# castacks/UniCeption

Hardware: AMD Instinct MI355X
Metric: image-pairs/sec fwd, ViT-L/16 two-view 512x512 (encoder + CroCo decoder + dpt heads + adaptor) (higher is better)
Workload: dtype bf16; 1 GPU; BASELINE configs[1]: ViT-L/16 CroCo encoder + 12-block CroCo decoder + dpt head, 512x512 pairs, forward, random-init weights; pairs_per_gpu=128, img=512, head=dpt, encoder=croco, attention=bf16, hipgraph=False, parallelism=dp1 (independent pairs per rank, no data-path collective)

## Files before the change

### uniception_amd/csrc/elementwise.hip

```cpp
#include "vec_access.h"
#include <type_traits>
#include "knobs.h"

template <typename TO>
__global__ void patch_gather_kernel(const float* __restrict__ img, typename TO::storage* __restrict__ cols, int B,
                                    int Cin, int H, int W, int P, int64_t items) {
    const int h = H / P, w = W / P;
    const int P4 = P / 4;
    for (int64_t it = (int64_t)blockIdx.x * blockDim.x + threadIdx.x; it < items; it += (int64_t)gridDim.x * blockDim.x) {
        int64_t r = it;
        const int v4 = (int)(r % P4); r /= P4;
        const int u = (int)(r % P); r /= P;
        const int c = (int)(r % Cin); r /= Cin;
        const int j = (int)(r % w); r /= w;
        const int i = (int)(r % h);
        const int b = (int)(r / h);
        const float4_t px = *reinterpret_cast<const float4_t*>(
            img + (((int64_t)b * Cin + c) * H + (int64_t)i * P + u) * W + (int64_t)j * P + v4 * 4);
        typename TO::storage* o = cols + it * 4;
        TO::store(o + 0, px.x); TO::store(o + 1, px.y); TO::store(o + 2, px.z); TO::store(o + 3, px.w);
    }
}

template <typename TO>
__global__ void patch_gather_scalar_kernel(const float* __restrict__ img, typename TO::storage* __restrict__ cols, int B,
                                           int Cin, int H, int W, int P, int64_t n) {
    const int h = H / P, w = W / P;
    for (int64_t it = (int64_t)blockIdx.x * blockDim.x + threadIdx.x; it < n; it += (int64_t)gridDim.x * blockDim.x) {
        int64_t r = it;
        const int v = (int)(r % P); r /= P;
        const int u = (int)(r % P); r /= P;
        const int c = (int)(r % Cin); r /= Cin;
        const int j = (int)(r % w); r /= w;
        const int i = (int)(r % h);
        const int b = (int)(r / h);
        TO::store(cols + it, img[(((int64_t)b * Cin + c) * H + (int64_t)i * P + u) * W + (int64_t)j * P + v]);
    }
}

extern "C" int uc_patch_gather(const float* img, void* cols, int out_dtype, int B, int Cin, int H, int W, int P,
                               uc_stream_t stream) {
    UC_REQUIRE(img && cols, "uc_patch_gather: null pointer");
    UC_REQUIRE(B > 0 && Cin > 0 && P > 0 && H % P == 0 && W % P == 0, "uc_patch_gather: H,W must be multiples of the patch size");
    hipStream_t st = (hipStream_t)stream;
    const bool quad = (P % 4 == 0) && (W % 4 == 0) && ((uintptr_t)img % 16 == 0);
    if (!quad) {
        const int64_t n = (int64_t)B * Cin * H * W;
        UC_DISPATCH("uc_patch_gather", out_dtype,
                    hipLaunchKernelGGL((patch_gather_scalar_kernel<Tag>), dim3(EW_GRID(n)), dim3(256), 0, st, img, (Tag::storage*)cols, B, Cin, H, W, P, n));
        UC_CHECK_LAUNCH("uc_patch_gather");
        return UC_OK;
    }
    const int64_t items = (int64_t)B * Cin * H * W / 4;
    UC_DISPATCH("uc_patch_gather", out_dtype,
                hipLaunchKernelGGL((patch_gather_kernel<Tag>), dim3(EW_GRID(items)), dim3(256), 0, st, img, (Tag::storage*)cols, B, Cin, H, W, P, items));
    UC_CHECK_LAUNCH("uc_patch_gather");
    return UC_OK;
}

template <typename TI, typename TO>
__global__ __launch_bounds__(256) void transpose2d_kernel(const typename TI::storage* __restrict__ src,
                                                          typename TO::storage* __restrict__ dst, int R, int S) {
    __shared__ float tile[32][33];
    const int64_t boff = (int64_t)blockIdx.z * R * S;
    const int s0 = blockIdx.x * 32, r0 = blockIdx.y * 32;
    const int tx = threadIdx.x & 31, ty = threadIdx.x >> 5;
#pragma unroll
    for (int k = 0; k < 4; ++k) {
        const int r = r0 + ty + 8 * k, s = s0 + tx;
        if (r < R && s < S) tile[ty + 8 * k][tx] = TI::load(src + boff + (int64_t)r * S + s);
    }
    __syncthreads();
#pragma unroll
    for (int k = 0; k < 4; ++k) {
        const int s = s0 + ty + 8 * k, r = r0 + tx;
        if (r < R && s < S) TO::store(dst + boff + (int64_t)s * R + r, tile[tx][ty + 8 * k]);
    }
}

template <typename TI, typename TO>
static void launch_transpose(const void* src, void* dst, int Bn, int R, int S, hipStream_t st) {
    hipLaunchKernelGGL((transpose2d_kernel<TI, TO>), dim3((S + 31) / 32, (R + 31) / 32, Bn), dim3(256), 0, st,
                       (const typename TI::storage*)src, (typename TO::storage*)dst, R, S);
}

static int dispatch_transpose(const char* name, const void* src, int sd, void* dst, int dd, int Bn, int R, int S,
                              hipStream_t st) {
    UC_REQUIRE(src && dst, "%s: null pointer", name);
    UC_REQUIRE(Bn > 0 && R > 0 && S > 0 && Bn <= 65535 && (R + 31) / 32 <= 65535, "%s: bad shape", name);
    if (sd == UC_F32 && dd == UC_F32) launch_transpose<F32Tag, F32Tag>(src, dst, Bn, R, S, st);
    else if (sd == UC_F32 && dd == UC_BF16) launch_transpose<F32Tag, BF16Tag>(src, dst, Bn, R, S, st);
    else if (sd == UC_BF16 && dd == UC_F32) launch_transpose<BF16Tag, F32Tag>(src, dst, Bn, R, S, st);
    else if (sd == UC_BF16 && dd == UC_BF16) launch_transpose<BF16Tag, BF16Tag>(src, dst, Bn, R, S, st);
    else if (sd == UC_F32 && dd == UC_F16) launch_transpose<F32Tag, F16Tag>(src, dst, Bn, R, S, st);
    else if (sd == UC_F16 && dd == UC_F32) launch_transpose<F16Tag, F32Tag>(src, dst, Bn, R, S, st);
    else if (sd == UC_BF16 && dd == UC_F16) launch_transpose<BF16Tag, F16Tag>(src, dst, Bn, R, S, st);
    else { uc_set_error("%s: unsupported dtypes %d -> %d", name, sd, dd); return UC_ERR_BAD_ARG; }
    UC_CHECK_LAUNCH(name);
    return UC_OK;
}

extern "C" int uc_nchw_to_nhwc(const void* src, int src_dtype, void* dst, int dst_dtype, int B, int C, int H, int W,
                               uc_stream_t stream) {
    return dispatch_transpose("uc_nchw_to_nhwc", src, src_dtype, dst, dst_dtype, B, C, H * W, (hipStream_t)stream);
}
extern "C" int uc_nhwc_to_nchw(const void* src, int src_dtype, void* dst, int dst_dtype, int B, int C, int H, int W,
                               uc_stream_t stream) {
    return dispatch_transpose("uc_nhwc_to_nchw", src, src_dtype, dst, dst_dtype, B, H * W, C, (hipStream_t)stream);
}

template <typename TI, typename TO>
__global__ void convert_kernel(const typename TI::storage* __restrict__ s, typename TO::storage* __restrict__ d, int64_t n, int* __restrict__ sat_flag, int vec) {
    constexpr bool TO_F16 = sizeof(typename TO::storage) == 2 && !std::is_same<TO, BF16Tag>::value;
    const int64_t n8 = vec ? n >> 3 : 0;
    float amax = 0.f;
    for (int64_t i = (int64_t)blockIdx.x * blockDim.x + threadIdx.x; i < n8; i += (int64_t)gridDim.x * blockDim.x) {
        float v[8];
        if constexpr (sizeof(typename TI::storage) == 4) {
            const float4_t a = *reinterpret_cast<const float4_t*>(s + i * 8), b = *reinterpret_cast<const float4_t*>(s + i * 8 + 4);
            v[0] = a.x; v[1] = a.y; v[2] = a.z; v[3] = a.w; v[4] = b.x; v[5] = b.y; v[6] = b.z; v[7] = b.w;
        } else {
            typename TI::storage raw[8];
            *reinterpret_cast<uint4*>(raw) = *reinterpret_cast<const uint4*>(s + i * 8);
#pragma unroll
            for (int k = 0; k < 8; ++k) v[k] = TI::load(raw + k);
        }
        if constexpr (TO_F16) {
#pragma unroll
            for (int k = 0; k < 8; ++k) amax = uc_amax(amax, fabsf(v[k]));
        }
        if constexpr (sizeof(typename TO::storage) == 4) {
            *reinterpret_cast<float4_t*>(d + i * 8) = (float4_t){v[0], v[1], v[2], v[3]};
            *reinterpret_cast<float4_t*>(d + i * 8 + 4) = (float4_t){v[4], v[5], v[6], v[7]};
        } else {
            typename TO::storage raw[8];
#pragma unroll
            for (int k = 0; k < 8; ++k) TO::store(raw + k, v[k]);
            *reinterpret_cast<uint4*>(d + i * 8) = *reinterpret_cast<const uint4*>(raw);
        }
    }
    for (int64_t i = (n8 << 3) + (int64_t)blockIdx.x * blockDim.x + threadIdx.x; i < n; i += (int64_t)gridDim.x * blockDim.x) {
        const float v = TI::load(s + i);
        if constexpr (TO_F16) amax = uc_amax(amax, fabsf(v));
        TO::store(d + i, v);
    }
    if constexpr (TO_F16) {
        if (sat_flag && !(amax <= UC_F16_MAX)) atomicOr(sat_flag, 1);
    }
}

extern "C" int uc_convert(const void* src, int sd, void* dst, int dd, int64_t n, int* sat_flag, uc_stream_t stream) {
    UC_REQUIRE(src && dst && n >= 0, "uc_convert: bad argument");
    if (n == 0) return UC_OK;
    const int vec = ((uintptr_t)src % 16 == 0 && (uintptr_t)dst % 16 == 0) ? 1 : 0;
    hipStream_t st = (hipStream_t)stream;
    const dim3 g(EW_GRID(vec ? (n + 7) / 8 : n)), b(256);
    if (sd == UC_F32 && dd == UC_BF16) hipLaunchKernelGGL((convert_kernel<F32Tag, BF16Tag>), g, b, 0, st, (const float*)src, (bf16_t*)dst, n, sat_flag, vec);
    else if (sd == UC_BF16 && dd == UC_F32) hipLaunchKernelGGL((convert_kernel<BF16Tag, F32Tag>), g, b, 0, st, (const bf16_t*)src, (float*)dst, n, sat_flag, vec);
    else if (sd == UC_F32 && dd == UC_F32) hipLaunchKernelGGL((convert_kernel<F32Tag, F32Tag>), g, b, 0, st, (const float*)src, (float*)dst, n, sat_flag, vec);
    else if (sd == UC_BF16 && dd == UC_BF16) hipLaunchKernelGGL((convert_kernel<BF16Tag, BF16Tag>), g, b, 0, st, (const bf16_t*)src, (bf16_t*)dst, n, sat_flag, vec);
    else if (sd == UC_F32 && dd == UC_F16) hipLaunchKernelGGL((convert_kernel<F32Tag, F16Tag>), g, b, 0, st, (const float*)src, (unsigned short*)dst, n, sat_flag, vec);
    else if (sd == UC_F16 && dd == UC_F32) hipLaunchKernelGGL((convert_kernel<F16Tag, F32Tag>), g, b, 0, st, (const unsigned short*)src, (float*)dst, n, sat_flag, vec);
    else if (sd == UC_BF16 && dd == UC_F16) hipLaunchKernelGGL((convert_kernel<BF16Tag, F16Tag>), g, b, 0, st, (const bf16_t*)src, (unsigned short*)dst, n, sat_flag, vec);
    else { uc_set_error("uc_convert: unsupported dtypes %d -> %d", sd, dd); return UC_ERR_BAD_ARG; }
    UC_CHECK_LAUNCH("uc_convert");
    return UC_OK;
}

__global__ void add_view_pe_kernel(float* __restrict__ x, const float* __restrict__ pe, int64_t B, int L, int T, int V, int C4) {
    const int64_t n = B * (int64_t)V * T * C4;
    for (int64_t i = (int64_t)blockIdx.x * blockDim.x + threadIdx.x; i < n; i += (int64_t)gridDim.x * blockDim.x) {
        const int c = (int)(i % C4);
        const int64_t r = i / C4;
        const int64_t bv = r / T;
        const int v = (int)(bv % V);
        const int64_t b = bv / V;
        float4_t* px = reinterpret_cast<float4_t*>(x + ((b * L + (int64_t)v * T + (r - bv * T)) * C4 + c) * 4);
        *px = *px + *reinterpret_cast<const float4_t*>(pe + ((int64_t)v * C4 + c) * 4);
    }
}

extern "C" int uc_add_view_pe(float* x, const float* pe, int64_t B, int L, int T, int V, int C, uc_stream_t stream) {
    UC_REQUIRE(x && pe && B >= 0 && L > 0 && T > 0 && V > 0 && (int64_t)V * T <= L && C > 0 && C % 4 == 0, "uc_add_view_pe: bad argument");
    UC_REQUIRE((uintptr_t)x % 16 == 0 && (uintptr_t)pe % 16 == 0, "uc_add_view_pe: 16-byte alignment");
    const int64_t n = B * (int64_t)V * T * (C / 4);
    if (n == 0) return UC_OK;
    hipLaunchKernelGGL(add_view_pe_kernel, dim3(EW_GRID(n)), dim3(256), 0, (hipStream_t)stream, x, pe, B, L, T, V, C / 4);
    UC_CHECK_LAUNCH("uc_add_view_pe");
    return UC_OK;
}

__global__ void split_bf16x3_kernel(const float* __restrict__ x, bf16_t* __restrict__ out, int64_t rows, int C8, int relu) {
    const int64_t n = rows * C8;
    for (int64_t i = (int64_t)blockIdx.x * blockDim.x + threadIdx.x; i < n; i += (int64_t)gridDim.x * blockDim.x) {
        const int64_t r = i / C8;
        const int c = (int)(i - r * C8);
        const float4_t* src = reinterpret_cast<const float4_t*>(x + (r * C8 + c) * 8);
        float v[8];
        const float4_t a = src[0], b = src[1];
        v[0] = a.x; v[1] = a.y; v[2] = a.z; v[3] = a.w; v[4] = b.x; v[5] = b.y; v[6] = b.z; v[7] = b.w;
        unsigned hi[4], lo[4];
#pragma unroll
        for (int k = 0; k < 4; ++k) {
            float p = v[2 * k], q = v[2 * k + 1];
            if (relu) { p = fmaxf(p, 0.f); q = fmaxf(q, 0.f); }
            const unsigned h = pack_bf16x2(p, q);
            hi[k] = h;
            lo[k] = pack_bf16x2(p - __uint_as_float(h << 16), q - __uint_as_float(h & 0xffff0000u));
        }
        bf16_t* dst = out + r * (int64_t)C8 * 24 + c * 8;
        const uint4 H = (uint4){hi[0], hi[1], hi[2], hi[3]};
        *reinterpret_cast<uint4*>(dst) = H;
        *reinterpret_cast<uint4*>(dst + (int64_t)C8 * 8) = H;
        *reinterpret_cast<uint4*>(dst + (int64_t)C8 * 16) = (uint4){lo[0], lo[1], lo[2], lo[3]};
    }
}

extern "C" int uc_split_bf16x3(const float* x, void* out, int64_t rows, int C, int relu, uc_stream_t stream) {
    UC_REQUIRE(x && out && rows >= 0 && C > 0 && C % 8 == 0, "uc_split_bf16x3: C must be a positive multiple of 8");
    UC_REQUIRE((uintptr_t)x % 16 == 0 && (uintptr_t)out % 16 == 0, "uc_split_bf16x3: 16-byte alignment");
    if (rows == 0) return UC_OK;
    const int64_t n = rows * (C / 8);
    hipLaunchKernelGGL(split_bf16x3_kernel, dim3(EW_GRID(n)), dim3(256), 0, (hipStream_t)stream, x, (bf16_t*)out, rows, C / 8, relu);
    UC_CHECK_LAUNCH("uc_split_bf16x3");
    return UC_OK;
}

template <typename Tag>
__global__ void bilinear_kernel(const typename Tag::storage* __restrict__ src, typename Tag::storage* __restrict__ dst,
                                int B, int Hi, int Wi, int C, int Ho, int Wo, int ch, int cw, float sy, float sx) {
    const unsigned C8 = (unsigned)C / 8u;
    const unsigned t = blockIdx.x * blockDim.x + threadIdx.x;
    if (t >= (unsigned)cw * C8) return;
    const unsigned ox = t / C8, c8 = t - ox * C8;
    const int oy = blockIdx.y, b = blockIdx.z;
    const float fy = sy * (float)oy, fx = sx * (float)ox;
    const int y0 = (int)fy, x0 = (int)fx;
    const int y1 = min(y0 + 1, Hi - 1), x1 = min(x0 + 1, Wi - 1);
    const float ly = fy - (float)y0, lx = fx - (float)x0;
    const float hy = 1.f - ly, hx = 1.f - lx;
    const typename Tag::storage* base = src + (int64_t)b * Hi * Wi * C + c8 * 8;
    const Vec8 p00 = vec_load8<Tag>(base + ((int64_t)y0 * Wi + x0) * C);
    const Vec8 p01 = vec_load8<Tag>(base + ((int64_t)y0 * Wi + x1) * C);
    const Vec8 p10 = vec_load8<Tag>(base + ((int64_t)y1 * Wi + x0) * C);
    const Vec8 p11 = vec_load8<Tag>(base + ((int64_t)y1 * Wi + x1) * C);
    Vec8 o;
#pragma unroll
    for (int e = 0; e < 8; ++e)
        o.v[e] = hy * (hx * p00.v[e] + lx * p01.v[e]) + ly * (hx * p10.v[e] + lx * p11.v[e]);
    vec_store8<Tag>(dst + (((int64_t)b * ch + oy) * cw) * C + (int64_t)t * 8, o);
}

template <typename Tag, int R>
__global__ void bilinear_rows_kernel(const typename Tag::storage* __restrict__ src, typename Tag::storage* __restrict__ dst,
                                     int B, int Hi, int Wi, int C, int Ho, int Wo, int ch, int cw, float sy, float sx) {
    constexpr int RIN = R / 2 + 2;
    const unsigned C8 = (unsigned)C / 8u;
    const unsigned t = blockIdx.x * blockDim.x + threadIdx.x;
    if (t >= (unsigned)cw * C8) return;
    const unsigned ox = t / C8, c8 = t - ox * C8;
    const int oy = R * blockIdx.y, b = blockIdx.z;
    const float fx = sx * (float)ox;
    const int x0 = (int)fx;
    const int x1 = min(x0 + 1, Wi - 1);
    const float lx = fx - (float)x0, hx = 1.f - lx;
    const int ya = (int)(sy * (float)oy);
    const typename Tag::storage* base = src + (int64_t)b * Hi * Wi * C + c8 * 8;
    float h[RIN][8];
#pragma unroll
    for (int i = 0; i < RIN; ++i) {
        const int64_t y = min(ya + i, Hi - 1);
        const Vec8 p0 = vec_load8<Tag>(base + (y * Wi + x0) * C), p1 = vec_load8<Tag>(base + (y * Wi + x1) * C);
#pragma unroll
        for (int e = 0; e < 8; ++e) h[i][e] = hx * p0.v[e] + lx * p1.v[e];
    }
#pragma unroll
    for (int k = 0; k < R; ++k) {
        if (oy + k >= ch) break;
        const float fy = sy * (float)(oy + k);
        const int y0 = (int)fy;
        const float ly = fy - (float)y0, hy = 1.f - ly;
        const int rel = y0 - ya;
        Vec8 o;
#pragma unroll
        for (int e = 0; e < 8; ++e) {
            float top = h[0][e], bot = h[1][e];
#pragma unroll
            for (int i = 1; i < RIN - 1; ++i) { top = rel == i ? h[i][e] : top; bot = rel == i ? h[i + 1][e] : bot; }
            o.v[e] = hy * top + ly * bot;
        }
        vec_store8<Tag>(dst + (((int64_t)b * ch + oy + k) * cw) * C + (int64_t)t * 8, o);
    }
}

extern "C" int uc_bilinear_nhwc(const void* src, void* dst, int dtype, int B, int Hi, int Wi, int C, int Ho, int Wo,
                                int crop_h, int crop_w, uc_stream_t stream) {
    UC_REQUIRE(src && dst, "uc_bilinear_nhwc: null pointer");
    UC_REQUIRE(B > 0 && Hi > 0 && Wi > 0 && Ho > 0 && Wo > 0 && C > 0 && C % 8 == 0, "uc_bilinear_nhwc: bad shape (C must be a multiple of 8)");
    UC_REQUIRE(crop_h > 0 && crop_h <= Ho && crop_w > 0 && crop_w <= Wo, "uc_bilinear_nhwc: bad crop");
    const float sy = Ho > 1 ? (float)(Hi - 1) / (float)(Ho - 1) : 0.f;
    const float sx = Wo > 1 ? (float)(Wi - 1) / (float)(Wo - 1) : 0.f;
    UC_REQUIRE(crop_h <= 65535 && B <= 65535 && (int64_t)crop_w * (C / 8) < ((int64_t)1 << 31), "uc_bilinear_nhwc: shape exceeds the launch grid");
    const dim3 grid((unsigned)(((int64_t)crop_w * (C / 8) + 255) / 256), (unsigned)crop_h, (unsigned)B);
    hipStream_t st = (hipStream_t)stream;
    const int rows2 = uc_knobs().bilinear_rows2;
    if (rows2 && sy <= 0.5f && (dtype == UC_BF16 || dtype == UC_F16)) {
#define UC_BL_ROWS(TAG, R)                                                                                                           \
    hipLaunchKernelGGL((bilinear_rows_kernel<TAG, R>), dim3(grid.x, (unsigned)((crop_h + R - 1) / R), (unsigned)B), dim3(256), 0, st, \
                       (const TAG::storage*)src, (TAG::storage*)dst, B, Hi, Wi, C, Ho, Wo, crop_h, crop_w, sy, sx)
        if (dtype == UC_F16) UC_BL_ROWS(F16Tag, 4);
        else if (rows2 == 4) UC_BL_ROWS(BF16Tag, 4);
        else UC_BL_ROWS(BF16Tag, 2);
#undef UC_BL_ROWS
        UC_CHECK_LAUNCH("uc_bilinear_nhwc");
        return UC_OK;
    }
    UC_DISPATCH_F16("uc_bilinear_nhwc", dtype,
                    hipLaunchKernelGGL((bilinear_kernel<Tag>), grid, dim3(256), 0, st, (const Tag::storage*)src, (Tag::storage*)dst, B, Hi, Wi, C, Ho, Wo, crop_h, crop_w, sy, sx));
    UC_CHECK_LAUNCH("uc_bilinear_nhwc");
    return UC_OK;
}

template <typename Tag>
__global__ void convt_scatter_kernel(const typename Tag::storage* __restrict__ src, typename Tag::storage* __restrict__ dst,
                                     int B, int h, int w, int k, int Cout, int64_t items) {
    const int C8 = Cout / 8;
    for (int64_t it = (int64_t)blockIdx.x * blockDim.x + threadIdx.x; it < items; it += (int64_t)gridDim.x * blockDim.x) {
        int64_t r = it;
        const int c8 = (int)(r % C8); r /= C8;
        const int X = (int)(r % (k * w)); r /= (k * w);
        const int Y = (int)(r % (k * h));
        const int b = (int)(r / (k * h));
        const int i = Y / k, u = Y % k, j = X / k, v = X % k;
        const int64_t srow = ((int64_t)b * h + i) * w + j;
        const Vec8 x = vec_load8<Tag>(src + srow * ((int64_t)k * k * Cout) + (int64_t)(u * k + v) * Cout + c8 * 8);
        vec_store8<Tag>(dst + it * 8, x);
    }
}

extern "C" int uc_convt_scatter(const void* src, void* dst, int dtype, int B, int h, int w, int k, int Cout,
                                uc_stream_t stream) {
    UC_REQUIRE(src && dst, "uc_convt_scatter: null pointer");
    UC_REQUIRE(B > 0 && h > 0 && w > 0 && k > 0 && Cout > 0 && Cout % 8 == 0, "uc_convt_scatter: bad shape (Cout must be a multiple of 8)");
    const int64_t items = (int64_t)B * h * w * k * k * (Cout / 8);
    hipStream_t st = (hipStream_t)stream;
    UC_DISPATCH_F16("uc_convt_scatter", dtype,
                    hipLaunchKernelGGL((convt_scatter_kernel<Tag>), dim3(EW_GRID(items)), dim3(256), 0, st, (const Tag::storage*)src, (Tag::storage*)dst, B, h, w, k, Cout, items));
    UC_CHECK_LAUNCH("uc_convt_scatter");
    return UC_OK;
}

template <typename Tag>
__global__ void pixel_shuffle_kernel(const typename Tag::storage* __restrict__ src, float* __restrict__ dst, int B, int h,
                                     int w, int P, int Cout, int64_t n) {
    const int Wd = P * w, Hd = P * h;
    for (int64_t it = (int64_t)blockIdx.x * blockDim.x + threadIdx.x; it < n; it += (int64_t)gridDim.x * blockDim.x) {
        int64_t r = it;
        const int X = (int)(r % Wd); r /= Wd;
        const int Y = (int)(r % Hd); r /= Hd;
        const int c = (int)(r % Cout);
        const int b = (int)(r / Cout);
        const int i = Y / P, u = Y % P, j = X / P, v = X % P;
        const int64_t srow = ((int64_t)b * h + i) * w + j;
        dst[it] = Tag::load(src + srow * ((int64_t)Cout * P * P) + (int64_t)c * P * P + u * P + v);
    }
}

extern "C" int uc_pixel_shuffle(const void* src, int src_dtype, float* dst, int B, int h, int w, int P, int Cout,
                                uc_stream_t stream) {
    UC_REQUIRE(src && dst && B > 0 && h > 0 && w > 0 && P > 0 && Cout > 0, "uc_pixel_shuffle: bad argument");
    const int64_t n = (int64_t)B * Cout * P * h * P * w;
    hipStream_t st = (hipStream_t)stream;
    UC_DISPATCH_F16("uc_pixel_shuffle", src_dtype,
                    hipLaunchKernelGGL((pixel_shuffle_kernel<Tag>), dim3(EW_GRID(n)), dim3(256), 0, st, (const Tag::storage*)src, dst, B, h, w, P, Cout, n));
    UC_CHECK_LAUNCH("uc_pixel_shuffle");
    return UC_OK;
}

__global__ void pointmap_adaptor_kernel(const float* __restrict__ x, int64_t sb, int64_t sc, int64_t sp,
                                        float* __restrict__ pts, float* __restrict__ conf, int64_t HW, int64_t n,
                                        float vmin, float vspan) {
    for (int64_t it = (int64_t)blockIdx.x * blockDim.x + threadIdx.x; it < n; it += (int64_t)gridDim.x * blockDim.x) {
        const int64_t b = it / HW, pix = it % HW;
        const float* px = x + b * sb + pix * sp;
        const float X = px[0], Y = px[sc], Z = px[2 * sc], Cf = px[3 * sc];
        const float d = sqrtf(X * X + Y * Y + Z * Z);
        const float s = expm1f(d) / fmaxf(d, 1e-8f);
        pts[it * 3 + 0] = X * s;
        pts[it * 3 + 1] = Y * s;
        pts[it * 3 + 2] = Z * s;
        conf[it] = vmin + fminf(expf(Cf), vspan);
    }
}

extern "C" int uc_pointmap_adaptor(const float* x, int64_t x_sb, int64_t x_sc, int64_t x_sp, float* pts, float* conf,
                                   int B, int H, int W, float conf_vmin, float conf_vmax, uc_stream_t stream) {
    UC_REQUIRE(x && pts && conf && B > 0 && H > 0 && W > 0, "uc_pointmap_adaptor: bad argument");
    const int64_t n = (int64_t)B * H * W;
    hipLaunchKernelGGL(pointmap_adaptor_kernel, dim3(EW_GRID(n)), dim3(256), 0, (hipStream_t)stream, x, x_sb, x_sc, x_sp,
                       pts, conf, (int64_t)H * W, n, conf_vmin, conf_vmax - conf_vmin);
    UC_CHECK_LAUNCH("uc_pointmap_adaptor");
    return UC_OK;
}

template <typename Tag>
__global__ __launch_bounds__(256) void conv1x1_to4_kernel(const typename Tag::storage* __restrict__ feat,
                                                          const float* __restrict__ w, const float* __restrict__ bias,
                                                          float* __restrict__ out, int64_t npix, int Cin) {
    __shared__ float ws[4][256];
    for (int i = threadIdx.x; i < 4 * Cin; i += blockDim.x) ws[i / Cin][i % Cin] = w[i];
    __syncthreads();
    for (int64_t pix = (int64_t)blockIdx.x * blockDim.x + threadIdx.x; pix < npix; pix += (int64_t)gridDim.x * blockDim.x) {
        float a0 = bias[0], a1 = bias[1], a2 = bias[2], a3 = bias[3];
        const typename Tag::storage* f = feat + pix * Cin;
        for (int c = 0; c < Cin; c += 8) {
            const Vec8 x = vec_load8<Tag>(f + c);
#pragma unroll
            for (int e = 0; e < 8; ++e) {
                a0 = fmaf(x.v[e], ws[0][c + e], a0);
                a1 = fmaf(x.v[e], ws[1][c + e], a1);
                a2 = fmaf(x.v[e], ws[2][c + e], a2);
                a3 = fmaf(x.v[e], ws[3][c + e], a3);
            }
        }
        *reinterpret_cast<float4_t*>(out + pix * 4) = (float4_t){a0, a1, a2, a3};
    }
}

template <typename Tag, int C8>
__global__ __launch_bounds__(256) void conv1x1_to4_coop_kernel(const typename Tag::storage* __restrict__ feat,
                                                               const float* __restrict__ w, const float* __restrict__ bias,
                                                               float* __restrict__ out, int64_t npix) {
    constexpr int Cin = C8 * 8;
    constexpr int PPB = 256 / C8;
    const int chunk = threadIdx.x % C8, pl = threadIdx.x / C8;
    float wr[4][8];
#pragma unroll
    for (int o = 0; o < 4; ++o)
#pragma unroll
        for (int e = 0; e < 8; ++e) wr[o][e] = w[o * Cin + chunk * 8 + e];
    const float4_t b4 = *reinterpret_cast<const float4_t*>(bias);
    for (int64_t pix = (int64_t)blockIdx.x * PPB + pl; pix < npix; pix += (int64_t)gridDim.x * PPB) {
        const Vec8 x = vec_load8<Tag>(feat + pix * Cin + chunk * 8);
        float a[4] = {0.f, 0.f, 0.f, 0.f};
#pragma unroll
        for (int e = 0; e < 8; ++e) {
            a[0] = fmaf(x.v[e], wr[0][e], a[0]);
            a[1] = fmaf(x.v[e], wr[1][e], a[1]);
            a[2] = fmaf(x.v[e], wr[2][e], a[2]);
            a[3] = fmaf(x.v[e], wr[3][e], a[3]);
        }
#pragma unroll
        for (int off = C8 / 2; off > 0; off >>= 1) {
#pragma unroll
            for (int o = 0; o < 4; ++o) a[o] += __shfl_xor(a[o], off, 64);
        }
        if (chunk == 0)
            *reinterpret_cast<float4_t*>(out + pix * 4) = (float4_t){a[0] + b4.x, a[1] + b4.y, a[2] + b4.z, a[3] + b4.w};
    }
}

template <typename Tag>
static bool launch_conv1x1_to4_coop(const void* feat, const float* w, const float* b, float* out, int64_t npix, int Cin, hipStream_t st) {
    const int C8 = Cin / 8;
// ... 366 lines not shown
```

### uniception_amd/csrc/error.hip

```cpp
#include "common.h"
#include "knobs.h"

#include <mutex>
#include <stdlib.h>
#include <string.h>

static thread_local char g_uc_err[512] = {0};

void uc_set_error(const char* fmt, ...) {
    va_list ap;
    va_start(ap, fmt);
    vsnprintf(g_uc_err, sizeof(g_uc_err), fmt, ap);
    va_end(ap);
}

extern "C" const char* uc_last_error(void) { return g_uc_err; }
extern "C" int uc_abi_version(void) { return UC_ABI_VERSION; }

#ifdef UC_DIAG
extern "C" const char* uc_build_flavor(void) { return "diag"; }
#else
extern "C" const char* uc_build_flavor(void) { return "release"; }
#endif

#define UC_ATTN_RS_DEFAULT 0
static UcKnobs g_knobs;
static std::once_flag g_knobs_once;
std::atomic<int> g_uc_gemm_variant{-3};
std::atomic<int> g_uc_gemm_stagger{-1};
std::atomic<int> g_uc_attn_rs{UC_ATTN_RS_DEFAULT};
std::atomic<int> g_uc_attn_p64{1};
std::atomic<int> g_uc_attn_bwd64{1};
std::atomic<int> g_uc_conv_rows{1};
std::atomic<int> g_uc_conv_rows_flat{1};
std::atomic<int> g_uc_small_m_split{2048};

static int env_int(const char* name, int dflt) {
    const char* e = getenv(name);
    return e ? atoi(e) : dflt;
}

const UcKnobs& uc_knobs() {
    std::call_once(g_knobs_once, [] {
        g_knobs.gemm_group_m = env_int("UC_GEMM_GROUP_M", 4);
        if (g_knobs.gemm_group_m < 1) g_knobs.gemm_group_m = 1;
        g_knobs.gemm_4wave = env_int("UC_GEMM_4WAVE", 3);
        g_knobs.attn_prio = env_int("UC_ATTN_PRIO", 0);
        g_knobs.bilinear_rows2 = env_int("UC_BILINEAR_ROWS2", 4);
        g_knobs.ln_nt = env_int("UC_LN_NT", -1);
#ifdef UC_DIAG
        g_knobs.gemm_dbg = env_int("UC_GEMM_DBG", 0);
        g_knobs.attn_dbg = env_int("UC_ATTN_DBG", 0);
        g_knobs.gemm_trace = env_int("UC_GEMM_TRACE", 0);
#endif
        g_uc_gemm_variant.store(env_int("UC_GEMM_VARIANT", -3));
        g_uc_gemm_stagger.store(env_int("UC_GEMM_STAGGER", -1));
        g_uc_attn_rs.store(env_int("UC_ATTN_RS", UC_ATTN_RS_DEFAULT));
        g_uc_attn_p64.store(env_int("UC_ATTN_P64", 1));
        g_uc_attn_bwd64.store(env_int("UC_ATTN_BWD64", 1));
        g_uc_conv_rows.store(env_int("UC_CONV_ROWS", 1));
        g_uc_conv_rows_flat.store(env_int("UC_CONV_ROWS_FLAT", 1));
        g_uc_small_m_split.store(env_int("UC_GEMM_SMALLM", 2048));
    });
    return g_knobs;
}

extern "C" int uc_tuning_set(const char* name, int value) {
    UC_REQUIRE(name, "uc_tuning_set: null name");
    (void)uc_knobs();
    if (!strcmp(name, "gemm_variant")) {
        UC_REQUIRE(value == -3 || value == -1 || (value >= 0 && value <= 4) || value == 6 || value == 7, "uc_tuning_set: gemm_variant must be -3 (automatic), -1, 0..4, 6 or 7 (got %d)", value);
        g_uc_gemm_variant.store(value);
    } else if (!strcmp(name, "gemm_stagger")) {
        UC_REQUIRE(value >= -1 && value <= 100000, "uc_tuning_set: gemm_stagger out of range (%d)", value);
        g_uc_gemm_stagger.store(value);
    } else if (!strcmp(name, "attn_role_split")) {
        UC_REQUIRE(value == 0 || value == 1, "uc_tuning_set: attn_role_split must be 0 or 1 (got %d)", value);
        g_uc_attn_rs.store(value);
    } else if (!strcmp(name, "attn_p64")) {
        UC_REQUIRE(value >= 0 && value <= 2, "uc_tuning_set: attn_p64 must be 0 (never), 1 (policy) or 2 (wherever the shape allows) (got %d)", value);
        g_uc_attn_p64.store(value);
    } else if (!strcmp(name, "attn_bwd64")) {
        UC_REQUIRE(value >= 0 && value <= 2, "uc_tuning_set: attn_bwd64 must be 0 (never), 1 (policy) or 2 (always) (got %d)", value);
        g_uc_attn_bwd64.store(value);
    } else if (!strcmp(name, "small_m_split")) {
        UC_REQUIRE(value >= 0, "uc_tuning_set: small_m_split is the smallest K a small-M launch splits in two for (0: never) (got %d)", value);
        g_uc_small_m_split.store(value);
    } else if (!strcmp(name, "conv_rows")) {
        UC_REQUIRE(value >= 0 && value <= 3, "uc_tuning_set: conv_rows must be 0 (implicit GEMM everywhere), 1 (row-walking kernels where they win), 2 (the 256-pixel row-walking kernel wherever the shape allows) or 3 (the eight-wave 512-pixel one wherever the shape allows) (got %d)", value);
        g_uc_conv_rows.store(value);
    } else if (!strcmp(name, "conv_rows_flat")) {
        UC_REQUIRE(value == 0 || value == 1, "uc_tuning_set: conv_rows_flat must be 0 (the eight-wave row kernel only on maps whose rows tile 512 pixels) or 1 (its flat form on every other map too) (got %d)", value);
        g_uc_conv_rows_flat.store(value);
    } else {
        uc_set_error("uc_tuning_set: unknown knob '%s' (run-time switchable: gemm_variant, gemm_stagger, attn_role_split, attn_p64, attn_bwd64, conv_rows, conv_rows_flat, small_m_split; everything else is read from the environment once, see csrc/knobs.h)", name);
        return UC_ERR_BAD_ARG;
    }
    return UC_OK;
}

extern "C" int uc_tuning_get(const char* name, int* value) {
    UC_REQUIRE(name && value, "uc_tuning_get: null argument");
    (void)uc_knobs();
    if (!strcmp(name, "gemm_variant")) *value = g_uc_gemm_variant.load();
    else if (!strcmp(name, "gemm_stagger")) *value = g_uc_gemm_stagger.load();
    else if (!strcmp(name, "attn_role_split")) *value = g_uc_attn_rs.load();
    else if (!strcmp(name, "attn_p64")) *value = g_uc_attn_p64.load();
    else if (!strcmp(name, "attn_bwd64")) *value = g_uc_attn_bwd64.load();
    else if (!strcmp(name, "conv_rows")) *value = g_uc_conv_rows.load();
    else if (!strcmp(name, "conv_rows_flat")) *value = g_uc_conv_rows_flat.load();
    else if (!strcmp(name, "small_m_split")) *value = g_uc_small_m_split.load();
    else { uc_set_error("uc_tuning_get: unknown knob '%s'", name); return UC_ERR_BAD_ARG; }
    return UC_OK;
}
```

### uniception_amd/csrc/knobs.h

```cpp
#pragma once
#include <atomic>

struct UcKnobs {
    int gemm_group_m;
    int gemm_4wave;
    int attn_prio;
    int bilinear_rows2;
    int ln_nt;
#ifdef UC_DIAG
    int gemm_dbg;
    int attn_dbg;
    int gemm_trace;
#endif
};
const UcKnobs& uc_knobs();

extern std::atomic<int> g_uc_gemm_variant;
extern std::atomic<int> g_uc_gemm_stagger;
extern std::atomic<int> g_uc_small_m_split;
extern std::atomic<int> g_uc_conv_rows;
extern std::atomic<int> g_uc_conv_rows_flat;
extern std::atomic<int> g_uc_attn_p64;
extern std::atomic<int> g_uc_attn_bwd64;
extern std::atomic<int> g_uc_attn_rs;

#ifdef UC_DIAG
#define UC_DBG(p, bits) ((p).dbg & (bits))
#define UC_TRACE(p) ((p).trace)
#else
#define UC_DBG(p, bits) (0)
#define UC_TRACE(p) ((unsigned long long*)nullptr)
#endif
```

### uniception_amd/csrc/vec_access.h

```cpp
#pragma once
#include "common.h"

struct Vec8 { float v[8]; };

__device__ __forceinline__ unsigned pack_f16x2(float lo, float hi) {
    const float2v_t v = {uc_sat_f16(lo), uc_sat_f16(hi)};
    return __builtin_bit_cast(unsigned, __builtin_convertvector(v, half2v_t));
}
__device__ __forceinline__ void unpack_f16x2(unsigned u, float& lo, float& hi) {
    const float2v_t v = __builtin_convertvector(__builtin_bit_cast(half2v_t, u), float2v_t);
    lo = v.x; hi = v.y;
}
__device__ __forceinline__ float4_t unpack_bf16x4(uint2 r) {
    return (float4_t){__uint_as_float(r.x << 16), __uint_as_float(r.x & 0xffff0000u), __uint_as_float(r.y << 16), __uint_as_float(r.y & 0xffff0000u)};
}

template <typename Tag> __device__ __forceinline__ Vec8 vec_load8(const typename Tag::storage* p);
template <> __device__ __forceinline__ Vec8 vec_load8<F32Tag>(const float* p) {
    Vec8 r;
    const float4_t a = *reinterpret_cast<const float4_t*>(p);
    const float4_t b = *reinterpret_cast<const float4_t*>(p + 4);
    r.v[0] = a.x; r.v[1] = a.y; r.v[2] = a.z; r.v[3] = a.w; r.v[4] = b.x; r.v[5] = b.y; r.v[6] = b.z; r.v[7] = b.w;
    return r;
}
template <> __device__ __forceinline__ Vec8 vec_load8<BF16Tag>(const bf16_t* p) {
    Vec8 r;
    const uint4 u = *reinterpret_cast<const uint4*>(p);
    r.v[0] = __uint_as_float(u.x << 16); r.v[1] = __uint_as_float(u.x & 0xffff0000u);
    r.v[2] = __uint_as_float(u.y << 16); r.v[3] = __uint_as_float(u.y & 0xffff0000u);
    r.v[4] = __uint_as_float(u.z << 16); r.v[5] = __uint_as_float(u.z & 0xffff0000u);
    r.v[6] = __uint_as_float(u.w << 16); r.v[7] = __uint_as_float(u.w & 0xffff0000u);
    return r;
}
template <> __device__ __forceinline__ Vec8 vec_load8<F16Tag>(const unsigned short* p) {
    Vec8 r;
    const uint4 u = *reinterpret_cast<const uint4*>(p);
    unpack_f16x2(u.x, r.v[0], r.v[1]); unpack_f16x2(u.y, r.v[2], r.v[3]);
    unpack_f16x2(u.z, r.v[4], r.v[5]); unpack_f16x2(u.w, r.v[6], r.v[7]);
    return r;
}

template <typename Tag> __device__ __forceinline__ void vec_store8(typename Tag::storage* p, const Vec8& r);
template <> __device__ __forceinline__ void vec_store8<F32Tag>(float* p, const Vec8& r) {
    *reinterpret_cast<float4_t*>(p) = (float4_t){r.v[0], r.v[1], r.v[2], r.v[3]};
    *reinterpret_cast<float4_t*>(p + 4) = (float4_t){r.v[4], r.v[5], r.v[6], r.v[7]};
}
template <> __device__ __forceinline__ void vec_store8<BF16Tag>(bf16_t* p, const Vec8& r) {
    uint4 u;
    u.x = pack_bf16x2(r.v[0], r.v[1]); u.y = pack_bf16x2(r.v[2], r.v[3]);
    u.z = pack_bf16x2(r.v[4], r.v[5]); u.w = pack_bf16x2(r.v[6], r.v[7]);
    *reinterpret_cast<uint4*>(p) = u;
}
template <> __device__ __forceinline__ void vec_store8<F16Tag>(unsigned short* p, const Vec8& r) {
    uint4 u;
    u.x = pack_f16x2(r.v[0], r.v[1]); u.y = pack_f16x2(r.v[2], r.v[3]);
    u.z = pack_f16x2(r.v[4], r.v[5]); u.w = pack_f16x2(r.v[6], r.v[7]);
    *reinterpret_cast<uint4*>(p) = u;
}

template <typename Tag> __device__ __forceinline__ float4_t vec_load4(const typename Tag::storage* p);
template <> __device__ __forceinline__ float4_t vec_load4<F32Tag>(const float* p) { return *reinterpret_cast<const float4_t*>(p); }
template <> __device__ __forceinline__ float4_t vec_load4<BF16Tag>(const bf16_t* p) { return unpack_bf16x4(*reinterpret_cast<const uint2*>(p)); }

template <typename Tag> __device__ __forceinline__ void vec_store4(typename Tag::storage* p, float4_t v);
template <> __device__ __forceinline__ void vec_store4<F32Tag>(float* p, float4_t v) { *reinterpret_cast<float4_t*>(p) = v; }
template <> __device__ __forceinline__ void vec_store4<BF16Tag>(bf16_t* p, float4_t v) {
    *reinterpret_cast<uint2*>(p) = (uint2){pack_bf16x2(v.x, v.y), pack_bf16x2(v.z, v.w)};
}

#define EW_GRID(n_items) ((unsigned)min((int64_t)65536 * 4, ceil_div64((n_items), 256)))

#define UC_REQUIRE_DTYPE(fn, dtype, F16)                                                                                    \
    UC_REQUIRE((dtype) == UC_F32 || (dtype) == UC_BF16 || ((F16) && (dtype) == UC_F16), "%s: unsupported dtype %d (%s)", fn, \
               dtype, (F16) ? "UC_F32, UC_BF16 or UC_F16" : "UC_F32 or UC_BF16")
#define UC_DISPATCH(fn, dtype, LAUNCH)                                              \
    do {                                                                            \
        UC_REQUIRE_DTYPE(fn, dtype, false);                                         \
        if ((dtype) == UC_F32) { typedef F32Tag Tag; LAUNCH; }                      \
        else { typedef BF16Tag Tag; LAUNCH; }                                       \
    } while (0)
#define UC_DISPATCH_F16(fn, dtype, LAUNCH)                                          \
    do {                                                                            \
        UC_REQUIRE_DTYPE(fn, dtype, true);                                          \
        if ((dtype) == UC_F32) { typedef F32Tag Tag; LAUNCH; }                      \
        else if ((dtype) == UC_BF16) { typedef BF16Tag Tag; LAUNCH; }               \
        else { typedef F16Tag Tag; LAUNCH; }                                        \
    } while (0)
```

Before: 396.6 image-pairs/s.

## Add LDS-staged band kernel for 2x bilinear upsampling in DPT head

Adds a bilinear band kernel, now the default path, in which each block stages a window of input rows and columns in shared memory. It then computes an 8-row by strip-wide output tile from that window and writes it with non-temporal stores when the output is large. The aim is to cut redundant global loads of source pixels across neighbouring output rows and columns, and to keep streaming output from polluting cache. It also remaps blocks across XCDs, makes the bilinear_rows2 knob switchable at run time, and rewrites the interpolation arithmetic as fmaf with contraction disabled, which can change results by rounding. Costs are LDS use that may lower occupancy, a sync per block, and host-side plan validation on every call.

```diff
diff --git a/uniception_amd/csrc/bilinear_plan.h b/uniception_amd/csrc/bilinear_plan.h
--- /dev/null
+++ b/uniception_amd/csrc/bilinear_plan.h
@@ -0,0 +1,71 @@
+#pragma once
+#include <stdint.h>
+
+static constexpr int UC_BL_BAND_ROWS = 8;
+static constexpr int UC_BL_BAND_CHUNKS = 512;
+static constexpr int UC_BL_BAND_LDS_MAX = 64 * 1024;
+static constexpr int64_t UC_BL_NT_BYTES = (int64_t)128 << 20;
+
+#ifdef __HIPCC__
+#define UC_BL_HD __host__ __device__
+#else
+#define UC_BL_HD
+#endif
+
+static inline float uc_bl_scale(int in, int out) { return out > 1 ? (float)(in - 1) / (float)(out - 1) : 0.f; }
+UC_BL_HD static inline int uc_bl_src0(float scale, int o) { return (int)(scale * (float)o); }
+
+struct BilinearBandPlan {
+    bool ok;
+    int rows, rows_in;
+    int strip, cols_in;
+    int nbands, nstrips;
+    int lds_bytes;
+    unsigned grid;
+    bool nt;
+};
+
+static inline BilinearBandPlan uc_bilinear_band_plan(int elem_bytes, int B, int Hi, int Wi, int C, int Ho, int Wo, int crop_h, int crop_w) {
+    BilinearBandPlan p = {};
+    const float sy = uc_bl_scale(Hi, Ho), sx = uc_bl_scale(Wi, Wo);
+    if (elem_bytes != 2 || C % 8 != 0 || sy > 0.5f || sx > 0.5f) return p;
+    const int C8 = C / 8;
+    p.rows = UC_BL_BAND_ROWS;
+    p.rows_in = p.rows / 2 + 2;
+    p.strip = (UC_BL_BAND_CHUNKS / C8) & ~1;
+    if (p.strip < 2) p.strip = 2;
+    p.cols_in = p.strip / 2 + 2;
+    const int64_t lds = (int64_t)p.rows_in * p.cols_in * C * 2;
+    if (lds > UC_BL_BAND_LDS_MAX) return p;
+    p.lds_bytes = (int)lds;
+    p.nbands = (crop_h + p.rows - 1) / p.rows;
+    p.nstrips = (crop_w + p.strip - 1) / p.strip;
+    const int64_t grid = (int64_t)B * p.nstrips * p.nbands;
+    if (grid >= ((int64_t)1 << 31)) return p;
+    p.grid = (unsigned)grid;
+    for (int b = 0; b < p.nbands; ++b) {
+        const int first = b * p.rows, last = (first + p.rows < crop_h ? first + p.rows : crop_h) - 1;
+        if (uc_bl_src0(sy, last) - uc_bl_src0(sy, first) > p.rows_in - 2) return p;
+    }
+    for (int s = 0; s < p.nstrips; ++s) {
+        const int first = s * p.strip, last = (first + p.strip < crop_w ? first + p.strip : crop_w) - 1;
+        if (uc_bl_src0(sx, last) - uc_bl_src0(sx, first) > p.cols_in - 2) return p;
+    }
+    p.nt = (int64_t)B * crop_h * crop_w * C * 2 > UC_BL_NT_BYTES;
+    p.ok = true;
+    return p;
+}
+
+struct BilinearBandTile { int b, oy, ox, rows, cols, ya, xa; };
+UC_BL_HD static inline BilinearBandTile uc_bilinear_band_tile(unsigned w, int nbands, int nstrips, int rows, int strip, int crop_h, int crop_w, float sy, float sx) {
+    BilinearBandTile t;
+    const unsigned bs = w / (unsigned)nbands;
+    t.b = (int)(bs / (unsigned)nstrips);
+    t.oy = (int)(w - bs * (unsigned)nbands) * rows;
+    t.ox = (int)(bs - (unsigned)t.b * (unsigned)nstrips) * strip;
+    t.rows = t.oy + rows < crop_h ? rows : crop_h - t.oy;
+    t.cols = t.ox + strip < crop_w ? strip : crop_w - t.ox;
+    t.ya = uc_bl_src0(sy, t.oy);
+    t.xa = uc_bl_src0(sx, t.ox);
+    return t;
+}
diff --git a/uniception_amd/csrc/elementwise.hip b/uniception_amd/csrc/elementwise.hip
--- a/uniception_amd/csrc/elementwise.hip
+++ b/uniception_amd/csrc/elementwise.hip
@@ -1,6 +1,8 @@
 #include "vec_access.h"
 #include <type_traits>
 #include "knobs.h"
+#include "mma_tile.h"
+#include "bilinear_plan.h"
 
 template <typename TO>
 __global__ void patch_gather_kernel(const float* __restrict__ img, typename TO::storage* __restrict__ cols, int B,
@@ -251,6 +253,41 @@
     vec_store8<Tag>(dst + (((int64_t)b * ch + oy) * cw) * C + (int64_t)t * 8, o);
 }
 
+__device__ __forceinline__ void bilinear_src(float scale, float o, int& i0, float& l) {
+#pragma clang fp contract(off)
+    i0 = (int)(scale * o);
+    l = fmaf(scale, o, -(float)i0);
+}
+__device__ __forceinline__ void bilinear_hrow(float hx, float lx, const Vec8& p0, const Vec8& p1, float (&h)[8]) {
+#pragma clang fp contract(off)
+#pragma unroll
+    for (int e = 0; e < 8; ++e) h[e] = fmaf(hx, p0.v[e], lx * p1.v[e]);
+}
+template <typename Tag, int R, bool NT>
+__device__ __forceinline__ void bilinear_vrows(const float (&h)[R / 2 + 2][8], int oy, int ya, int ch, float sy, typename Tag::storage* out, int64_t row_stride) {
+#pragma clang fp contract(off)
+    constexpr int RIN = R / 2 + 2;
+#pragma unroll
+    for (int k = 0; k < R; ++k) {
+        if (oy + k >= ch) break;
+        int y0;
+        float ly;
+        bilinear_src(sy, (float)(oy + k), y0, ly);
+        const float hy = 1.f - ly;
+        const int rel = y0 - ya;
+        Vec8 o;
+#pragma unroll
+        for (int e = 0; e < 8; ++e) {
+            float top = h[0][e], bot = h[1][e];
+#pragma unroll
+            for (int i = 1; i < RIN - 1; ++i) { top = rel == i ? h[i][e] : top; bot = rel == i ? h[i + 1][e] : bot; }
+            o.v[e] = fmaf(hy, top, ly * bot);
+        }
+        if constexpr (NT) vec_store8_nt<Tag>(out + k * row_stride, o);
+        else vec_store8<Tag>(out + k * row_stride, o);
+    }
+}
+
 template <typename Tag, int R>
 __global__ void bilinear_rows_kernel(const typename Tag::storage* __restrict__ src, typename Tag::storage* __restrict__ dst,
                                      int B, int Hi, int Wi, int C, int Ho, int Wo, int ch, int cw, float sy, float sx) {
@@ -260,36 +297,57 @@
     if (t >= (unsigned)cw * C8) return;
     const unsigned ox = t / C8, c8 = t - ox * C8;
     const int oy = R * blockIdx.y, b = blockIdx.z;
-    const float fx = sx * (float)ox;
-    const int x0 = (int)fx;
+    int x0;
+    float lx;
+    bilinear_src(sx, (float)ox, x0, lx);
     const int x1 = min(x0 + 1, Wi - 1);
-    const float lx = fx - (float)x0, hx = 1.f - lx;
+    const float hx = 1.f - lx;
     const int ya = (int)(sy * (float)oy);
     const typename Tag::storage* base = src + (int64_t)b * Hi * Wi * C + c8 * 8;
     float h[RIN][8];
 #pragma unroll
     for (int i = 0; i < RIN; ++i) {
         const int64_t y = min(ya + i, Hi - 1);
-        const Vec8 p0 = vec_load8<Tag>(base + (y * Wi + x0) * C), p1 = vec_load8<Tag>(base + (y * Wi + x1) * C);
-#pragma unroll
-        for (int e = 0; e < 8; ++e) h[i][e] = hx * p0.v[e] + lx * p1.v[e];
-    }
-#pragma unroll
-    for (int k = 0; k < R; ++k) {
-        if (oy + k >= ch) break;
-        const float fy = sy * (float)(oy + k);
-        const int y0 = (int)fy;
-        const float ly = fy - (float)y0, hy = 1.f - ly;
-        const int rel = y0 - ya;
-        Vec8 o;
-#pragma unroll
-        for (int e = 0; e < 8; ++e) {
-            float top = h[0][e], bot = h[1][e];
-#pragma unroll
-            for (int i = 1; i < RIN - 1; ++i) { top = rel == i ? h[i][e] : top; bot = rel == i ? h[i + 1][e] : bot; }
-            o.v[e] = hy * top + ly * bot;
-        }
-        vec_store8<Tag>(dst + (((int64_t)b * ch + oy + k) * cw) * C + (int64_t)t * 8, o);
+        bilinear_hrow(hx, lx, vec_load8<Tag>(base + (y * Wi + x0) * C), vec_load8<Tag>(base + (y * Wi + x1) * C), h[i]);
+    }
+    bilinear_vrows<Tag, R, false>(h, oy, ya, ch, sy, dst + (((int64_t)b * ch + oy) * cw) * C + (int64_t)t * 8, (int64_t)cw * C);
+}
+
+template <typename Tag, int R, bool NT>
+__global__ __launch_bounds__(256) void bilinear_band_kernel(const typename Tag::storage* __restrict__ src, typename Tag::storage* __restrict__ dst,
+                                                            int Hi, int Wi, int C8, int ch, int cw, float sy, float sx, int strip, int cols_in,
+                                                            int nbands, int nstrips, uc_fastdiv dC8) {
+    constexpr int RIN = R / 2 + 2;
+    extern __shared__ uint4 band_win[];
+    const BilinearBandTile t = uc_bilinear_band_tile((unsigned)xcd_remap((int)blockIdx.x, (int)gridDim.x), nbands, nstrips, R, strip, ch, cw, sy, sx);
+    const int b = t.b, oy = t.oy, ox0 = t.ox, ya = t.ya, xa = t.xa;
+    const int C = C8 * 8;
+    const int row_chunks = min(cols_in, Wi - xa) * C8;
+    const uint4* img = reinterpret_cast<const uint4*>(src + (int64_t)b * Hi * Wi * C);
+    for (int j = threadIdx.x; j < row_chunks; j += 256) {
+        uint4 v[RIN];
+#pragma unroll
+        for (int i = 0; i < RIN; ++i) v[i] = img[((int64_t)min(ya + i, Hi - 1) * Wi + xa) * C8 + j];
+#pragma unroll
+        for (int i = 0; i < RIN; ++i) band_win[i * cols_in * C8 + j] = v[i];
+    }
+    __syncthreads();
+    const typename Tag::storage* win = reinterpret_cast<const typename Tag::storage*>(band_win);
+    typename Tag::storage* out = dst + (((int64_t)b * ch + oy) * cw + ox0) * C;
+    const int items = t.cols * C8;
+    for (int it = threadIdx.x; it < items; it += 256) {
+        const unsigned oxr = uc_div((unsigned)it, dC8), c8 = (unsigned)it - oxr * (unsigned)C8;
+        int x0;
+        float lx;
+        bilinear_src(sx, (float)((unsigned)ox0 + oxr), x0, lx);
+        const int x1 = min(x0 + 1, Wi - 1);
+        const float hx = 1.f - lx;
+        const int o0 = ((x0 - xa) * C8 + (int)c8) * 8, o1 = ((x1 - xa) * C8 + (int)c8) * 8;
+        float h[RIN][8];
+#pragma unroll
+        for (int i = 0; i < RIN; ++i)
+            bilinear_hrow(hx, lx, vec_load8<Tag>(win + i * cols_in * C + o0), vec_load8<Tag>(win + i * cols_in * C + o1), h[i]);
+        bilinear_vrows<Tag, R, NT>(h, oy, ya, ch, sy, out + (int64_t)it * 8, (int64_t)cw * C);
     }
 }
 
@@ -298,18 +356,33 @@
     UC_REQUIRE(src && dst, "uc_bilinear_nhwc: null pointer");
     UC_REQUIRE(B > 0 && Hi > 0 && Wi > 0 && Ho > 0 && Wo > 0 && C > 0 && C % 8 == 0, "uc_bilinear_nhwc: bad shape (C must be a multiple of 8)");
     UC_REQUIRE(crop_h > 0 && crop_h <= Ho && crop_w > 0 && crop_w <= Wo, "uc_bilinear_nhwc: bad crop");
-    const float sy = Ho > 1 ? (float)(Hi - 1) / (float)(Ho - 1) : 0.f;
-    const float sx = Wo > 1 ? (float)(Wi - 1) / (float)(Wo - 1) : 0.f;
+    const float sy = uc_bl_scale(Hi, Ho), sx = uc_bl_scale(Wi, Wo);
     UC_REQUIRE(crop_h <= 65535 && B <= 65535 && (int64_t)crop_w * (C / 8) < ((int64_t)1 << 31), "uc_bilinear_nhwc: shape exceeds the launch grid");
     const dim3 grid((unsigned)(((int64_t)crop_w * (C / 8) + 255) / 256), (unsigned)crop_h, (unsigned)B);
     hipStream_t st = (hipStream_t)stream;
-    const int rows2 = uc_knobs().bilinear_rows2;
+    (void)uc_knobs();
+    const int rows2 = g_uc_bilinear_rows2.load(std::memory_order_relaxed);
+    if (rows2 == 8 && (dtype == UC_BF16 || dtype == UC_F16)) {
+        const BilinearBandPlan p = uc_bilinear_band_plan(2, B, Hi, Wi, C, Ho, Wo, crop_h, crop_w);
+        if (p.ok) {
+#define UC_BL_BAND(TAG, R, NT)                                                                                                                 \
+    hipLaunchKernelGGL((bilinear_band_kernel<TAG, R, NT>), dim3(p.grid), dim3(256), p.lds_bytes, st, (const TAG::storage*)src, (TAG::storage*)dst, \
+                       Hi, Wi, C / 8, crop_h, crop_w, sy, sx, p.strip, p.cols_in, p.nbands, p.nstrips, uc_make_fastdiv((unsigned)(C / 8)))
+#define UC_BL_BAND_NT(TAG, R) do { if (p.nt) UC_BL_BAND(TAG, R, true); else UC_BL_BAND(TAG, R, false); } while (0)
+            if (dtype == UC_F16) UC_BL_BAND_NT(F16Tag, UC_BL_BAND_ROWS);
+            else UC_BL_BAND_NT(BF16Tag, UC_BL_BAND_ROWS);
+#undef UC_BL_BAND_NT
+#undef UC_BL_BAND
+            UC_CHECK_LAUNCH("uc_bilinear_nhwc");
+            return UC_OK;
+        }
+    }
     if (rows2 && sy <= 0.5f && (dtype == UC_BF16 || dtype == UC_F16)) {
 #define UC_BL_ROWS(TAG, R)                                                                                                           \
     hipLaunchKernelGGL((bilinear_rows_kernel<TAG, R>), dim3(grid.x, (unsigned)((crop_h + R - 1) / R), (unsigned)B), dim3(256), 0, st, \
                        (const TAG::storage*)src, (TAG::storage*)dst, B, Hi, Wi, C, Ho, Wo, crop_h, crop_w, sy, sx)
         if (dtype == UC_F16) UC_BL_ROWS(F16Tag, 4);
-        else if (rows2 == 4) UC_BL_ROWS(BF16Tag, 4);
+        else if (rows2 != 2) UC_BL_ROWS(BF16Tag, 4);
         else UC_BL_ROWS(BF16Tag, 2);
 #undef UC_BL_ROWS
         UC_CHECK_LAUNCH("uc_bilinear_nhwc");
diff --git a/uniception_amd/csrc/error.hip b/uniception_amd/csrc/error.hip
--- a/uniception_amd/csrc/error.hip
+++ b/uniception_amd/csrc/error.hip
@@ -34,6 +34,7 @@
 std::atomic<int> g_uc_conv_rows{1};
 std::atomic<int> g_uc_conv_rows_flat{1};
 std::atomic<int> g_uc_small_m_split{2048};
+std::atomic<int> g_uc_bilinear_rows2{8};
 
 static int env_int(const char* name, int dflt) {
     const char* e = getenv(name);
@@ -46,7 +47,6 @@
         if (g_knobs.gemm_group_m < 1) g_knobs.gemm_group_m = 1;
         g_knobs.gemm_4wave = env_int("UC_GEMM_4WAVE", 3);
         g_knobs.attn_prio = env_int("UC_ATTN_PRIO", 0);
-        g_knobs.bilinear_rows2 = env_int("UC_BILINEAR_ROWS2", 4);
         g_knobs.ln_nt = env_int("UC_LN_NT", -1);
 #ifdef UC_DIAG
         g_knobs.gemm_dbg = env_int("UC_GEMM_DBG", 0);
@@ -61,6 +61,7 @@
         g_uc_conv_rows.store(env_int("UC_CONV_ROWS", 1));
         g_uc_conv_rows_flat.store(env_int("UC_CONV_ROWS_FLAT", 1));
         g_uc_small_m_split.store(env_int("UC_GEMM_SMALLM", 2048));
+        g_uc_bilinear_rows2.store(env_int("UC_BILINEAR_ROWS2", 8));
     });
     return g_knobs;
 }
@@ -92,8 +93,11 @@
     } else if (!strcmp(name, "conv_rows_flat")) {
         UC_REQUIRE(value == 0 || value == 1, "uc_tuning_set: conv_rows_flat must be 0 (the eight-wave row kernel only on maps whose rows tile 512 pixels) or 1 (its flat form on every other map too) (got %d)", value);
         g_uc_conv_rows_flat.store(value);
+    } else if (!strcmp(name, "bilinear_rows2")) {
+        UC_REQUIRE(value == 0 || value == 2 || value == 4 || value == 8, "uc_tuning_set: bilinear_rows2 must be 8 (band kernel), 4 or 2 (rows per work item of the row kernel) or 0 (one-row kernel) (got %d)", value);
+        g_uc_bilinear_rows2.store(value);
     } else {
-        uc_set_error("uc_tuning_set: unknown knob '%s' (run-time switchable: gemm_variant, gemm_stagger, attn_role_split, attn_p64, attn_bwd64, conv_rows, conv_rows_flat, small_m_split; everything else is read from the environment once, see csrc/knobs.h)", name);
+        uc_set_error("uc_tuning_set: unknown knob '%s' (run-time switchable: gemm_variant, gemm_stagger, attn_role_split, attn_p64, attn_bwd64, conv_rows, conv_rows_flat, small_m_split, bilinear_rows2; everything else is read from the environment once, see csrc/knobs.h)", name);
         return UC_ERR_BAD_ARG;
     }
     return UC_OK;
@@ -110,6 +114,7 @@
     else if (!strcmp(name, "conv_rows")) *value = g_uc_conv_rows.load();
     else if (!strcmp(name, "conv_rows_flat")) *value = g_uc_conv_rows_flat.load();
     else if (!strcmp(name, "small_m_split")) *value = g_uc_small_m_split.load();
+    else if (!strcmp(name, "bilinear_rows2")) *value = g_uc_bilinear_rows2.load();
     else { uc_set_error("uc_tuning_get: unknown knob '%s'", name); return UC_ERR_BAD_ARG; }
     return UC_OK;
 }
diff --git a/uniception_amd/csrc/knobs.h b/uniception_amd/csrc/knobs.h
--- a/uniception_amd/csrc/knobs.h
+++ b/uniception_amd/csrc/knobs.h
@@ -5,7 +5,6 @@
     int gemm_group_m;
     int gemm_4wave;
     int attn_prio;
-    int bilinear_rows2;
     int ln_nt;
 #ifdef UC_DIAG
     int gemm_dbg;
@@ -22,6 +21,7 @@
 extern std::atomic<int> g_uc_conv_rows_flat;
 extern std::atomic<int> g_uc_attn_p64;
 extern std::atomic<int> g_uc_attn_bwd64;
+extern std::atomic<int> g_uc_bilinear_rows2;
 extern std::atomic<int> g_uc_attn_rs;
 
 #ifdef UC_DIAG
diff --git a/uniception_amd/csrc/vec_access.h b/uniception_amd/csrc/vec_access.h
--- a/uniception_amd/csrc/vec_access.h
+++ b/uniception_amd/csrc/vec_access.h
@@ -45,17 +45,23 @@
     *reinterpret_cast<float4_t*>(p) = (float4_t){r.v[0], r.v[1], r.v[2], r.v[3]};
     *reinterpret_cast<float4_t*>(p + 4) = (float4_t){r.v[4], r.v[5], r.v[6], r.v[7]};
 }
-template <> __device__ __forceinline__ void vec_store8<BF16Tag>(bf16_t* p, const Vec8& r) {
+template <typename Tag> __device__ __forceinline__ uint4 vec_pack8(const Vec8& r);
+template <> __device__ __forceinline__ uint4 vec_pack8<BF16Tag>(const Vec8& r) {
     uint4 u;
     u.x = pack_bf16x2(r.v[0], r.v[1]); u.y = pack_bf16x2(r.v[2], r.v[3]);
     u.z = pack_bf16x2(r.v[4], r.v[5]); u.w = pack_bf16x2(r.v[6], r.v[7]);
-    *reinterpret_cast<uint4*>(p) = u;
+    return u;
 }
-template <> __device__ __forceinline__ void vec_store8<F16Tag>(unsigned short* p, const Vec8& r) {
+template <> __device__ __forceinline__ uint4 vec_pack8<F16Tag>(const Vec8& r) {
     uint4 u;
     u.x = pack_f16x2(r.v[0], r.v[1]); u.y = pack_f16x2(r.v[2], r.v[3]);
     u.z = pack_f16x2(r.v[4], r.v[5]); u.w = pack_f16x2(r.v[6], r.v[7]);
-    *reinterpret_cast<uint4*>(p) = u;
+    return u;
+}
+template <> __device__ __forceinline__ void vec_store8<BF16Tag>(bf16_t* p, const Vec8& r) { *reinterpret_cast<uint4*>(p) = vec_pack8<BF16Tag>(r); }
+template <> __device__ __forceinline__ void vec_store8<F16Tag>(unsigned short* p, const Vec8& r) { *reinterpret_cast<uint4*>(p) = vec_pack8<F16Tag>(r); }
+template <typename Tag> __device__ __forceinline__ void vec_store8_nt(typename Tag::storage* p, const Vec8& r) {
+    __builtin_nontemporal_store(__builtin_bit_cast(float4_t, vec_pack8<Tag>(r)), reinterpret_cast<float4_t*>(p));
 }
 
 template <typename Tag> __device__ __forceinline__ float4_t vec_load4(const typename Tag::storage* p);
```

Result: no change. 398.1 image-pairs/s (median of 6 runs) (+0.4%).
